# themayflyman/yet-another-raytracer

Hardware: NVIDIA B200
Metric: Mrays/s (primary+secondary) on david.obj 1920x1080 max-depth 50 (higher is better)
Workload: dtype f64

## Files before the change

### yet-another-raytracer_b200/csrc/device_trace.cuh

```cuda
#pragma once
#include "device_common.cuh"

namespace yart {

#ifndef YART_TRACE_THREADS
#define YART_TRACE_THREADS 128
#endif
constexpr int kTraceThreads = YART_TRACE_THREADS;
constexpr uint32_t kSentinel = 0x7FFFFFFFu;


YART_DEV bool sphere_t(D3 center, double radius, D3 ro, D3 rd, double t_min, double t_max, double& t) {
  D3 oc = ro - center;
  double a = length_squared(rd);
  double half_b = dot(oc, rd);
  double c = length_squared(oc) - radius * radius;
  double disc = half_b * half_b - a * c;
  if (disc < 0.0) return false;
  t = (0.0 - half_b - sqrt(disc)) / a;
  if (t < t_min || t_max < t) {
    t = (0.0 - half_b + sqrt(disc)) / a;
    if (t < t_min || t_max < t) return false;
  }
  return true;
// ... 219 lines not shown
  const float4* nodes;
  const float4* tris;
  const float4* leafgeo;
  const uint4* cnodes;
  float corigin[3], cscale;
  uint32_t root;
  uint32_t obj_index;
  uint32_t wrap;
  uint32_t refill_threshold;
  uint32_t node_threshold;
  uint32_t _pad;
  uint32_t n_nodes, n_tris;
  double sin_theta, cos_theta, offset[3];
  double bound[3];
  uint32_t* work_counter;
  unsigned long long* counters;
};

struct AnalyticParams {
  PassCommon c;
  DevScene scene;
  const yart_object* objects;
  uint32_t obj_begin, obj_end;
  const double* ray_time;
  uint64_t seed;
  uint32_t bounce;
  uint32_t spp_batch;
  uint32_t sample_base;
  uint32_t pixel_base;
  uint32_t media_mask;
  uint32_t _pad;
};

YART_DEV double min_nn(double a, double b) { return a < b ? a : b; }
YART_DEV double max_nn(double a, double b) { return a > b ? a : b; }

template <bool NEAR>
__device__ __noinline__ uint32_t box4_ieee(const float4* nd, double ox, double oy, double oz, double ix, double iy,
                                           double iz, double t_min, double t_best) {
  const float4 mnx = __ldg(nd + 0), mny = __ldg(nd + 2), mnz = __ldg(nd + 4);
  const float4 mxx = __ldg(nd + 1), mxy = __ldg(nd + 3), mxz = __ldg(nd + 5);
  uint32_t hitmask = 0;
#define YART_BOX(K, LX, LY, LZ, HX, HY, HZ)                                        \
  {                                                                                \
    double t0 = ((double)(LX) - ox) * ix, t1 = ((double)(HX) - ox) * ix;           \
    double tn = fmax(t_min, fmin(t0, t1));                                         \
    double tf = fmin(NEAR ? d_inf() : t_best, fmax(t0, t1));                       \
    t0 = ((double)(LY) - oy) * iy; t1 = ((double)(HY) - oy) * iy;                  \
    tn = fmax(tn, fmin(t0, t1)); tf = fmin(tf, fmax(t0, t1));                      \
    t0 = ((double)(LZ) - oz) * iz; t1 = ((double)(HZ) - oz) * iz;                  \
    tn = fmax(tn, fmin(t0, t1)); tf = fmin(tf, fmax(t0, t1));                      \
    const bool h = NEAR ? ((tf > tn) && (t_best >= tn)) : (tf > tn);               \
    hitmask |= h ? (1u << (K)) : 0u;                                               \
  }
  YART_BOX(0, mnx.x, mny.x, mnz.x, mxx.x, mxy.x, mxz.x)
  YART_BOX(1, mnx.y, mny.y, mnz.y, mxx.y, mxy.y, mxz.y)
  YART_BOX(2, mnx.z, mny.z, mnz.z, mxx.z, mxy.z, mxz.z)
  YART_BOX(3, mnx.w, mny.w, mnz.w, mxx.w, mxy.w, mxz.w)
#undef YART_BOX
  return hitmask;
}

#ifndef YART_TRAVERSE_MIN_BLOCKS
#define YART_TRAVERSE_MIN_BLOCKS 4
#endif

// ... 95 lines not shown
        }
        cur_used = 0;
        nxt_stage = 0;
        nxt_cnt = 0;
        if (!dyn_done) {
          if (lane == 0) claim_raw = atomicAdd(P.work_counter, 32u);
          nxt_stage = 1;
        }
        const uint32_t rank2 = rank - take1;
        const uint32_t take2 = min(need - take1, cur_cnt);
        const uint32_t id2 = __shfl_sync(0xffffffffu, id_cur, rank2 & 31u);
        if (fetching && !got && rank2 < take2) {
          new_id = id2;
          got = true;
        }
        cur_used = take2;
        if (fetching && !got) exhausted = true;
      } else if (nxt_stage == 1) {
        const uint64_t nb = dyn_base + __shfl_sync(0xffffffffu, claim_raw, 0);
        nxt_cnt = nb < n_items ? (uint32_t)min((unsigned long long)32, (unsigned long long)(n_items - nb)) : 0u;
        id_nxt = YART_MISS;
        if (lane < nxt_cnt) id_nxt = P.c.queue ? P.c.queue[nb + lane] : (uint32_t)(nb + lane);
        if (nxt_cnt < 32u) dyn_done = true;
        nxt_stage = 2;
      }
      if (got) {
        {
          ray_id = new_id;
          YART_CHECK(ray_id < P.c.n_rays);
          D3 ro, rd;
          if (P.c.rays32) load_ray_f32(P.c.rays32 + ray_id, ro, rd);
          else load_ray(P.c.rays + ray_id, ro, rd);
          t_best = P.c.first_pass ? P.c.t_max : fmin(P.c.hits[ray_id].t, P.c.t_max);
          if (NEAR) t_best = just_below(t_best);
          if (P.wrap & YART_WRAP_TRANSLATE) ro = ro - d3(P.offset[0], P.offset[1], P.offset[2]);
          if (P.wrap & YART_WRAP_ROTATE_Y) {
            const double ct = P.cos_theta, st = P.sin_theta;
            D3 org = ro, dir = rd;
            org.x = ct * ro.x - st * ro.z;
            org.z = st * ro.x + ct * ro.z;
            dir.x = ct * rd.x - st * rd.z;
            dir.z = st * rd.x + ct * rd.z;
            ro = org;
            rd = dir;
          }
          ox = ro.x; oy = ro.y; oz = ro.z;
          dx = rd.x; dy = rd.y; dz = rd.z;
          ix = 1.0 / dx; iy = 1.0 / dy; iz = 1.0 / dz;
          pos = (dx >= 0.0 ? 1u : 0u) | (dy >= 0.0 ? 2u : 0u) | (dz >= 0.0 ? 4u : 0u);
          sgn = NEAR ? (pos ^ 7u) : pos;
          if (!(isfinite(ix) && isfinite(iy) && isfinite(iz) && isfinite(ox) && isfinite(oy) && isfinite(oz))) pos |= 8u;
          if (MIXED) {
            ixf = (float)ix; iyf = (float)iy; izf = (float)iz;
            cxf = (float)(-(ox * ix)); cyf = (float)(-(oy * iy)); czf = (float)(-(oz * iz));
            const double a = fmax(fmax((P.bound[0] + fabs(ox)) * fabs(ix), (P.bound[1] + fabs(oy)) * fabs(iy)),
                                  (P.bound[2] + fabs(oz)) * fabs(iz));
            amax2 = __double2float_ru(a * (1.0 / 4194304.0));
            const float lo = 1e-30f, hi = 1e30f;
            const bool ok = fabsf(ixf) > lo && fabsf(ixf) < hi && fabsf(iyf) > lo && fabsf(iyf) < hi && fabsf(izf) > lo &&
                            fabsf(izf) < hi && fabsf(cxf) < hi && fabsf(cyf) < hi && fabsf(czf) < hi && amax2 < hi;
            if (!ok) pos |= 8u;
            t_best_f = (float)t_best;
          }
          cur = P.root;
          sp = 0;
          best_prim = YART_MISS;
          best_bu = best_bv = 0.0;
// ... 180 lines not shown
    YART_CHECK(ray_id < P.c.n_rays);
    D3 wo, wd;
    if (P.c.rays32) load_ray_f32(P.c.rays32 + ray_id, wo, wd);
    else load_ray(P.c.rays + ray_id, wo, wd);
    DevHit h;
    if (P.c.first_pass) {
      h.t = d_inf(); h.bu = 0.0; h.bv = 0.0; h.obj = YART_MISS; h.prim = 0;
    } else {
      h = P.c.hits[ray_id];
    }
    double t_best = fmin(h.t, P.c.t_max);
    bool changed = P.c.first_pass != 0;
    Rng rng;
    if (P.media_mask) rng = make_rng(P.seed, P.pixel_base + ray_id / P.spp_batch, P.sample_base + ray_id % P.spp_batch);
    else rng = make_rng(0, 0, 0);
    const double time = P.ray_time ? P.ray_time[ray_id] : 0.0;
    for (uint32_t oi = P.obj_begin; oi < P.obj_end; ++oi) {
      const yart_object& o = P.objects[oi];
      double t, bu = 0.0, bv = 0.0;
      uint32_t prim = 0;
      bool hit;
      if (o.kind == YART_OBJ_SPHERE && o.wrap == 0)
        hit = sphere_t(d3(o.p[0], o.p[1], o.p[2]), o.p[3], wo, wd, P.c.t_min, t_best, t);
      else
        hit = object_hit_t(P.scene, o, oi, wo, wd, time, P.c.t_min, t_best, rng, P.bounce, t, prim, bu, bv);
      if (hit) {
        t_best = t; h.t = t; h.obj = oi; h.prim = prim; h.bu = bu; h.bv = bv;
        changed = true;
      }
    }
    if (changed) P.c.hits[ray_id] = h;
  }
}
#endif

}
```

### yet-another-raytracer_b200/csrc/device_trace_lean.cu

```cuda
#define YART_TRACE_NO_ANALYTIC_KERNEL
#include "device_trace.cuh"

namespace yart {

template <bool NEAR, int STACK, int MIN_BLOCKS, bool COMPACT>
__global__ void __launch_bounds__(kTraceThreads, MIN_BLOCKS) k_traverse_lean(const TraverseParams P) {
  constexpr bool MIXED = true;
  __shared__ uint32_t s_stack[STACK + 1][kTraceThreads];
  __shared__ double s_ray[6][kTraceThreads];
  __shared__ double s_buv[2][kTraceThreads];
  const int tid = threadIdx.x;
  const uint32_t lane = tid & 31;
  const uint32_t n_items = P.c.n_items_dev ? *P.c.n_items_dev : (uint32_t)P.c.n_items;
  const uint32_t warp_global = (blockIdx.x * kTraceThreads + tid) >> 5;
  const uint32_t total_warps = gridDim.x * (kTraceThreads / 32);
  const uint32_t rpw = max(1u, min(32u, (uint32_t)(((uint64_t)n_items + total_warps - 1) / total_warps)));
  const uint32_t dyn_base = total_warps * rpw;
  if ((uint64_t)warp_global * rpw >= n_items) return;
  const uint32_t cur_base = warp_global * rpw;
  struct {
    uint32_t cur_cnt : 6, cur_used : 6, nxt_cnt : 6, nxt_stage : 2, dyn_done : 1;
  } w;
  w.cur_cnt = min(rpw, n_items - cur_base);
  w.cur_used = 0;
// ... 80 lines not shown
        }
        w.cur_used = 0;
        w.nxt_stage = 0;
        w.nxt_cnt = 0;
        if (!w.dyn_done) {
          if (lane == 0) claim_raw = atomicAdd(P.work_counter, 32u);
          w.nxt_stage = 1;
        }
        const uint32_t rank2 = rank - take1;
        const uint32_t take2 = min(need - take1, (uint32_t)w.cur_cnt);
        const uint32_t id2 = __shfl_sync(0xffffffffu, id_cur, rank2 & 31u);
        if (fetching && !got && rank2 < take2) {
          new_id = id2;
          got = true;
        }
        w.cur_used = take2;
        if (fetching && !got) exhausted = true;
      } else if (w.nxt_stage == 1) {
        const uint64_t nb = (uint64_t)dyn_base + __shfl_sync(0xffffffffu, claim_raw, 0);
        w.nxt_cnt = nb < n_items ? min(32u, n_items - (uint32_t)nb) : 0u;
        id_nxt = YART_MISS;
        if (lane < w.nxt_cnt) id_nxt = P.c.queue ? P.c.queue[nb + lane] : (uint32_t)(nb + lane);
        if (w.nxt_cnt < 32u) w.dyn_done = 1;
        w.nxt_stage = 2;
      }
      if (got) {
        {
          ray_id = new_id;
          YART_CHECK(ray_id < P.c.n_rays);
          D3 ro, rd;
          if (P.c.rays32) load_ray_f32(P.c.rays32 + ray_id, ro, rd);
          else load_ray(P.c.rays + ray_id, ro, rd);
          t_best = P.c.first_pass ? P.c.t_max : fmin(P.c.hits[ray_id].t, P.c.t_max);
          if (NEAR) t_best = just_below(t_best);
          if (P.wrap & YART_WRAP_TRANSLATE) ro = ro - d3(P.offset[0], P.offset[1], P.offset[2]);
          if (P.wrap & YART_WRAP_ROTATE_Y) {
            const double ct = P.cos_theta, st = P.sin_theta;
            D3 org = ro, dir = rd;
            org.x = ct * ro.x - st * ro.z;
            org.z = st * ro.x + ct * ro.z;
            dir.x = ct * rd.x - st * rd.z;
            dir.z = st * rd.x + ct * rd.z;
            ro = org;
            rd = dir;
          }
          const double ox = ro.x, oy = ro.y, oz = ro.z, dx = rd.x, dy = rd.y, dz = rd.z;
          const double ix = 1.0 / dx, iy = 1.0 / dy, iz = 1.0 / dz;
          s_ray[0][tid] = ox; s_ray[1][tid] = oy; s_ray[2][tid] = oz;
          s_ray[3][tid] = dx; s_ray[4][tid] = dy; s_ray[5][tid] = dz;
          pos = (dx >= 0.0 ? 1u : 0u) | (dy >= 0.0 ? 2u : 0u) | (dz >= 0.0 ? 4u : 0u);
          sgn = NEAR ? (pos ^ 7u) : pos;
          if (!(isfinite(ix) && isfinite(iy) && isfinite(iz) && isfinite(ox) && isfinite(oy) && isfinite(oz))) pos |= 8u;
          if (MIXED) {
            ixf = (float)ix; iyf = (float)iy; izf = (float)iz;
            cxf = (float)(-(ox * ix)); cyf = (float)(-(oy * iy)); czf = (float)(-(oz * iz));
            const double a = fmax(fmax((P.bound[0] + fabs(ox)) * fabs(ix), (P.bound[1] + fabs(oy)) * fabs(iy)),
                                  (P.bound[2] + fabs(oz)) * fabs(iz));
            amax2 = __double2float_ru(a * (1.0 / 4194304.0));
            const float lo = 1e-30f, hi = 1e30f;
            const bool ok = fabsf(ixf) > lo && fabsf(ixf) < hi && fabsf(iyf) > lo && fabsf(iyf) < hi && fabsf(izf) > lo &&
                            fabsf(izf) < hi && fabsf(cxf) < hi && fabsf(cyf) < hi && fabsf(czf) < hi && amax2 < hi;
            if (!ok) pos |= 8u;
            if (COMPACT) {
              const float ax = P.cscale * ixf, ay = P.cscale * iyf, az = P.cscale * izf;
              const float bx = fmaf(-8388608.f, ax, fmaf(P.corigin[0], ixf, cxf));
              const float by = fmaf(-8388608.f, ay, fmaf(P.corigin[1], iyf, cyf));
              const float bz = fmaf(-8388608.f, az, fmaf(P.corigin[2], izf, czf));
// ... 242 lines not shown
```

### yet-another-raytracer_b200/csrc/yart_device.cu

```cuda
#include <algorithm>
#include <cfloat>
#include <cmath>
#include <cstdio>
#include <cstdlib>
#include <cstring>
#include <map>
#include <numeric>
#include <string>
#include <vector>

#include "../../include/yart_spectral_tables.h"
#include "device_build.h"
#include "device_shade.cuh"
#include "host_common.h"

namespace yart {

__global__ void __launch_bounds__(256) k_export(const DevScene S, const yart_ray* rays, const DevHit* hits, yart_hit* out_hits,
                                                 uint64_t n) {
  for (uint64_t i = blockIdx.x * (uint64_t)blockDim.x + threadIdx.x; i < n; i += (uint64_t)gridDim.x * blockDim.x) {
    const DevHit h = hits[i];
    yart_hit out;
    if (h.obj == YART_MISS) {
      out.t = d_inf(); out.u = 0.0; out.v = 0.0; out.prim_id = YART_MISS; out.obj_id = YART_MISS; out.front_face = 0;
// ... 299 lines not shown
    nd.pad[0] = nd.pad[1] = nd.pad[2] = 0;
    nodes.push_back(nd);
    id = (uint32_t)nodes.size() - 1;
    return merge(merge(bx[0], bx[1]), merge(bx[2], bx[3]));
  }
};

}
}

using namespace yart;

struct yart_ctx {
  int device = 0;
  int sm_count = 148;
  cudaStream_t stream = nullptr;
  bool own_stream = true;
  std::string err;

  bool have_scene = false;
  std::vector<void*> scene_allocs;
  DevScene scene;
  yart_object* d_solo = nullptr;
  std::map<const void*, int> traverse_blocks;
  std::vector<yart_object> h_objects;
  std::vector<DevMesh> h_meshes;
  uint32_t n_meshes = 0;
  uint32_t max_stack = 0;
  bool has_media = false;
  uint32_t builder = YART_BUILDER_DEVICE;
  double* d_cie = nullptr;
  double* d_smits = nullptr;

  DevBuf rays, hits_export, time, wavelength, throughput, hits, queue_a, queue_b, counts, work, counters, film, rgba;
  cudaEvent_t ev0 = nullptr, ev1 = nullptr;
  std::vector<cudaEvent_t> ev_pool;
  cudaStream_t copy_in = nullptr, copy_out = nullptr;
  std::vector<cudaEvent_t> chunk_events;

  void free_scene() {
    for (void* p : scene_allocs) cudaFree(p);
    scene_allocs.clear();
    have_scene = false;
    d_solo = nullptr;
  }
};

namespace yart {
cudaStream_t ctx_stream(yart_ctx* ctx) { return ctx->stream; }
int ctx_device(const yart_ctx* ctx) { return ctx->device; }
void ctx_set_error(yart_ctx* ctx, const std::string& msg) { ctx->err = msg; }
}

namespace {

template <class T>
int upload(yart_ctx* ctx, const T* host, size_t n, T** out) {
  *out = nullptr;
  if (n == 0) return YART_OK;
  void* p = nullptr;
  CUDA_TRY(ctx, cudaMalloc(&p, n * sizeof(T)));
  ctx->scene_allocs.push_back(p);
  CUDA_TRY(ctx, cudaMemcpyAsync(p, host, n * sizeof(T), cudaMemcpyHostToDevice, ctx->stream));
  *out = reinterpret_cast<T*>(p);
  return YART_OK;
}

DevCamera make_camera(const yart_camera& c) {
  auto sub = [](const double* a, const double* b, double* o) { for (int i = 0; i < 3; ++i) o[i] = a[i] - b[i]; };
  auto unit = [](double* a) {
    double l = std::sqrt(a[0] * a[0] + a[1] * a[1] + a[2] * a[2]);
// ... 34 lines not shown

typedef void (*TraverseKernel)(const TraverseParams);
}
namespace yart {
TraverseKernel lean_traverse_kernel(bool near, uint32_t max_stack, int ctas_per_sm, bool compact);
}
namespace {
template <bool MIXED>
TraverseKernel pick_traverse_kernel_m(bool near, bool count, uint32_t max_stack) {
  if (max_stack <= 32) {
    if (near) return count ? k_traverse<true, true, 32, MIXED> : k_traverse<true, false, 32, MIXED>;
    return count ? k_traverse<false, true, 32, MIXED> : k_traverse<false, false, 32, MIXED>;
  }
  if (near) return count ? k_traverse<true, true, 64, MIXED> : k_traverse<true, false, 64, MIXED>;
  return count ? k_traverse<false, true, 64, MIXED> : k_traverse<false, false, 64, MIXED>;
}
TraverseKernel pick_traverse_kernel(bool near, bool count, uint32_t max_stack, bool mixed) {
  return mixed ? pick_traverse_kernel_m<true>(near, count, max_stack) : pick_traverse_kernel_m<false>(near, count, max_stack);
}

struct QueryArgs {
  PassCommon c;
  const yart_object* d_objects;
  const yart_object* h_objects;
  uint32_t n_objects;
  const double* ray_time;
  uint64_t seed;
  uint32_t bounce, spp_batch, sample_base, pixel_base;
  uint32_t* work_counters;
  unsigned long long* counters;
  bool near, count;
};

int run_passes(yart_ctx* ctx, const QueryArgs& q, uint64_t* launches) {
  static const int rt = tune_env("YART_TUNE_RT", 8), nt = tune_env("YART_TUNE_NT", 12);
  static const int carve = tune_env("YART_TUNE_CARVEOUT", 35);
  static const int carve_lean = tune_env("YART_TUNE_CARVEOUT_LEAN", 50);
  static const int mixed = tune_env("YART_TUNE_MIXED", 1);
  bool first = true;
  uint32_t i = 0, n_trav = 0;
  auto is_mesh = [&](uint32_t k) {
    return q.h_objects[k].kind == YART_OBJ_MESH && !(q.h_objects[k].wrap & YART_WRAP_MEDIUM);
  };
  if (q.n_objects == 0) {
    AnalyticParams A;
    memset(&A, 0, sizeof(A));
    A.c = q.c;
    A.c.first_pass = 1;
    A.scene = ctx->scene;
    A.objects = q.d_objects;
    A.spp_batch = 1;
    k_analytic<<<ctx->sm_count * 8, 256, 0, ctx->stream>>>(A);
    if (launches) (*launches)++;
  }
  while (i < q.n_objects) {
    if (is_mesh(i)) {
      const yart_object& o = q.h_objects[i];
      const DevMesh& m = ctx->h_meshes[o.index];
      TraverseParams T;
      memset(&T, 0, sizeof(T));
      T.c = q.c;
      T.c.first_pass = first ? 1u : 0u;
      T.nodes = m.nodes;
      T.tris = m.tris;
      T.leafgeo = m.leafgeo;
      T.cnodes = m.cnodes;
      T.cscale = m.cscale;
      for (int k = 0; k < 3; ++k) T.corigin[k] = m.corigin[k];
      T.root = m.root;
      T.n_nodes = m.n_nodes;
      T.n_tris = m.n_tris;
      T.obj_index = i;
      T.wrap = o.wrap & (YART_WRAP_ROTATE_Y | YART_WRAP_TRANSLATE);
      T.refill_threshold = (uint32_t)std::max(1, std::min(32, rt));
      T.node_threshold = (uint32_t)std::max(1, std::min(32, nt));
      T.sin_theta = o.sin_theta;
      T.cos_theta = o.cos_theta;
      for (int k = 0; k < 3; ++k) T.offset[k] = o.offset[k];
      T.work_counter = q.work_counters + n_trav++;
      T.counters = q.counters;
      for (int k = 0; k < 3; ++k) T.bound[k] = m.bound[k];
      static const int lean = tune_env("YART_TUNE_LEAN", 5);
      static const int lean_stack24 = tune_env("YART_TUNE_LEAN_STACK24", 1);
      static const int lean_ref = tune_env("YART_TUNE_LEAN_REF", 0);
      const bool use_lean = lean && mixed && !q.count && (q.near || lean_ref);
      TraverseKernel k = use_lean ? yart::lean_traverse_kernel(q.near, (lean_stack24 || ctx->max_stack > 24) ? ctx->max_stack : 25u, lean,
                                                                 m.cnodes != nullptr && q.near)
                                  : pick_traverse_kernel(q.near, q.count, ctx->max_stack, mixed != 0);
      int& per_sm = ctx->traverse_blocks[(const void*)k];
      if (per_sm == 0) {
        cudaFuncSetAttribute(reinterpret_cast<const void*>(k), cudaFuncAttributePreferredSharedMemoryCarveout, use_lean ? carve_lean : carve);
        CUDA_TRY(ctx, cudaOccupancyMaxActiveBlocksPerMultiprocessor(&per_sm, reinterpret_cast<const void*>(k), kTraceThreads, 0));
        per_sm = std::max(per_sm, 1);
      }
      k<<<per_sm * ctx->sm_count, kTraceThreads, 0, ctx->stream>>>(T);
      i++;
    } else {
      uint32_t j = i;
      while (j < q.n_objects && !is_mesh(j)) ++j;
      AnalyticParams A;
      memset(&A, 0, sizeof(A));
      A.c = q.c;
      A.c.first_pass = first ? 1u : 0u;
      A.scene = ctx->scene;
      A.objects = q.d_objects;
      A.obj_begin = i;
      A.obj_end = j;
      A.ray_time = q.ray_time;
      A.seed = q.seed;
      A.bounce = q.bounce;
      A.spp_batch = q.spp_batch ? q.spp_batch : 1;
      A.sample_base = q.sample_base;
      A.pixel_base = q.pixel_base;
      A.media_mask = ctx->has_media ? 1u : 0u;
      k_analytic<<<ctx->sm_count * 8, 256, 0, ctx->stream>>>(A);
      i = j;
    }
    first = false;
    if (launches) (*launches)++;
  }
  CUDA_TRY(ctx, cudaGetLastError());
  return YART_OK;
}

}

extern "C" {

int yart_device_count(void) {
  int n = 0;
  if (cudaGetDeviceCount(&n) != cudaSuccess) return 0;
  return n;
}

int yart_ctx_create(int device, yart_ctx** out) {
  if (!out) {
    set_global_error("yart_ctx_create: null argument");
    return YART_ERR_INVALID;
  }
  int n = 0;
  cudaError_t e = cudaGetDeviceCount(&n);
  if (e != cudaSuccess || n <= 0) {
    set_global_error(std::string("no CUDA device: ") + (e != cudaSuccess ? cudaGetErrorString(e) : "device count is 0") +
                     " (this library has no CPU fallback)");
    return YART_ERR_CUDA;
  }
  if (device < 0 || device >= n) {
    set_global_error("yart_ctx_create: device index out of range");
    return YART_ERR_INVALID;
  }
  cudaDeviceProp prop;
  if ((e = cudaSetDevice(device)) != cudaSuccess || (e = cudaGetDeviceProperties(&prop, device)) != cudaSuccess) {
// ... 4 lines not shown
    set_global_error("this library is built for sm_100a (B200) only; device is sm_" + std::to_string(prop.major) +
                     std::to_string(prop.minor));
    return YART_ERR_CUDA;
  }
  yart_ctx* ctx = new yart_ctx();
  ctx->device = device;
  ctx->sm_count = prop.multiProcessorCount;
  if ((e = cudaStreamCreateWithFlags(&ctx->stream, cudaStreamNonBlocking)) != cudaSuccess ||
      (e = cudaEventCreate(&ctx->ev0)) != cudaSuccess || (e = cudaEventCreate(&ctx->ev1)) != cudaSuccess ||
      (e = cudaMalloc((void**)&ctx->d_cie, sizeof(double) * 3 * YART_N_CIE)) != cudaSuccess ||
      (e = cudaMalloc((void**)&ctx->d_smits, sizeof(double) * 7 * YART_N_BINS)) != cudaSuccess) {
    set_global_error(std::string("context setup: ") + cudaGetErrorString(e));
    delete ctx;
    return YART_ERR_CUDA;
  }
  if ((e = cudaMemcpy(ctx->d_cie, YART_CIE_X, sizeof(double) * YART_N_CIE, cudaMemcpyHostToDevice)) != cudaSuccess ||
      (e = cudaMemcpy(ctx->d_cie + YART_N_CIE, YART_CIE_Y, sizeof(double) * YART_N_CIE, cudaMemcpyHostToDevice)) != cudaSuccess ||
      (e = cudaMemcpy(ctx->d_cie + 2 * YART_N_CIE, YART_CIE_Z, sizeof(double) * YART_N_CIE, cudaMemcpyHostToDevice)) != cudaSuccess ||
      (e = cudaMemcpy(ctx->d_smits, YART_SMITS_BASIS, sizeof(double) * 7 * YART_N_BINS, cudaMemcpyHostToDevice)) != cudaSuccess) {
    set_global_error(std::string("context setup (spectral tables): ") + cudaGetErrorString(e));
    yart_ctx_destroy(ctx);
    return YART_ERR_CUDA;
  }
  *out = ctx;
  return YART_OK;
}

void yart_ctx_destroy(yart_ctx* ctx) {
  if (!ctx) return;
  cudaSetDevice(ctx->device);
  cudaDeviceSynchronize();
  ctx->free_scene();
  DevBuf* bufs[] = {&ctx->rays, &ctx->hits_export, &ctx->time, &ctx->wavelength, &ctx->throughput, &ctx->hits,
                    &ctx->queue_a, &ctx->queue_b, &ctx->counts, &ctx->work, &ctx->counters, &ctx->film, &ctx->rgba};
  for (DevBuf* b : bufs) b->release();
  for (cudaEvent_t e : ctx->ev_pool) cudaEventDestroy(e);
  for (cudaEvent_t e : ctx->chunk_events) cudaEventDestroy(e);
  if (ctx->copy_in) cudaStreamDestroy(ctx->copy_in);
  if (ctx->copy_out) cudaStreamDestroy(ctx->copy_out);
  if (ctx->ev0) cudaEventDestroy(ctx->ev0);
  if (ctx->ev1) cudaEventDestroy(ctx->ev1);
  if (ctx->d_cie) cudaFree(ctx->d_cie);
  if (ctx->d_smits) cudaFree(ctx->d_smits);
  if (ctx->own_stream && ctx->stream) cudaStreamDestroy(ctx->stream);
  delete ctx;
}

const char* yart_last_error(const yart_ctx* ctx) { return ctx ? ctx->err.c_str() : yart_last_error_global(); }

int yart_ctx_set_stream(yart_ctx* ctx, void* cuda_stream) {
  if (!ctx) return YART_ERR_INVALID;
  CUDA_TRY(ctx, cudaSetDevice(ctx->device));
  if (ctx->stream || !ctx->own_stream) CUDA_TRY(ctx, cudaStreamSynchronize(ctx->stream));
  if (ctx->own_stream && ctx->stream) cudaStreamDestroy(ctx->stream);
  ctx->stream = reinterpret_cast<cudaStream_t>(cuda_stream);
  ctx->own_stream = false;
  return YART_OK;
}

int yart_host_register(yart_ctx* ctx, void* ptr, uint64_t bytes) {
  if (!ctx) return YART_ERR_INVALID;
  if (!ptr || !bytes) {
    ctx->err = "yart_host_register: null pointer or zero size";
    return YART_ERR_INVALID;
  }
  CUDA_TRY(ctx, cudaSetDevice(ctx->device));
  const cudaError_t e = cudaHostRegister(ptr, (size_t)bytes, cudaHostRegisterPortable);
  if (e != cudaSuccess) {
    cudaGetLastError();
    ctx->err = std::string("yart_host_register: ") + cudaGetErrorString(e);
// ... 378 lines not shown
  const char* fn = f32 ? "yart_closest_hit_f32" : "yart_closest_hit";
  if (!ctx->have_scene) {
    ctx->err = std::string(fn) + ": no scene (call yart_ctx_set_scene first)";
    return YART_ERR_INVALID;
  }
  if ((n && (!rays || !hits)) || n > 0xFFFFFFF0ull || order > YART_ORDER_NEAR) {
    ctx->err = std::string(fn) + ": bad argument";
    return YART_ERR_INVALID;
  }
  const uintptr_t ray_align = f32 ? 7u : 15u, hit_align = f32 ? 3u : 7u;
  if ((flags & YART_FLAG_DEVICE_PTRS) && ((reinterpret_cast<uintptr_t>(rays) & ray_align) || (reinterpret_cast<uintptr_t>(hits) & hit_align))) {
    ctx->err = std::string(fn) + (f32 ? ": device ray arrays must be 8-byte aligned (hits: 4)" : ": device ray arrays must be 16-byte aligned (hits: 8)");
    return YART_ERR_INVALID;
  }
  if (target != YART_TARGET_WORLD && target >= ctx->n_meshes) {
    ctx->err = std::string(fn) + ": target is neither a mesh index nor YART_TARGET_WORLD";
    return YART_ERR_INVALID;
  }
  CUDA_TRY(ctx, cudaSetDevice(ctx->device));
  if (stats) memset(stats, 0, sizeof(*stats));
  if (n == 0) return YART_OK;
  const size_t ray_bytes = f32 ? sizeof(yart_ray_f32) : sizeof(yart_ray), hit_bytes = f32 ? sizeof(yart_hit_f32) : sizeof(yart_hit);
  const bool dev = (flags & YART_FLAG_DEVICE_PTRS) != 0;
  const bool count = (flags & YART_FLAG_COUNT_VISITS) != 0;
  const char* d_rays = static_cast<const char*>(rays);
  char* d_hits = static_cast<char*>(hits);
  if (!dev) {
    CUDA_TRY(ctx, ctx->rays.reserve(n * ray_bytes));
    CUDA_TRY(ctx, ctx->hits_export.reserve(n * hit_bytes));
    d_rays = ctx->rays.as<char>();
    d_hits = ctx->hits_export.as<char>();
  }
  const uint32_t n_list = (target == YART_TARGET_WORLD) ? ctx->scene.n_objects : 1u;
  const size_t work_bytes = ((size_t)n_list + 2) * sizeof(uint32_t);
  CUDA_TRY(ctx, ctx->work.reserve(work_bytes));
  CUDA_TRY(ctx, ctx->counters.reserve(64));
  CUDA_TRY(ctx, ctx->hits.reserve(n * sizeof(DevHit)));
  CUDA_TRY(ctx, cudaMemsetAsync(ctx->counters.p, 0, 64, ctx->stream));

  yart_object solo;
  memset(&solo, 0, sizeof(solo));
  solo.kind = YART_OBJ_MESH;
  solo.cos_theta = 1.0;
  QueryArgs q;
  memset(&q, 0, sizeof(q));
  q.c.t_min = t_min;
  q.c.t_max = t_max;
  DevScene export_scene = ctx->scene;
  if (target == YART_TARGET_WORLD) {
    q.d_objects = ctx->scene.objects;
    q.h_objects = ctx->h_objects.data();
    q.n_objects = ctx->scene.n_objects;
  } else {
    solo.index = target;
    q.d_objects = ctx->d_solo + target;
    q.h_objects = &solo;
    q.n_objects = 1;
    export_scene.objects = ctx->d_solo + target;
  }
  q.seed = 0;
  q.bounce = 1;
  q.spp_batch = 1;
  q.work_counters = ctx->work.as<uint32_t>();
  q.counters = ctx->counters.as<unsigned long long>();
  q.near = order == YART_ORDER_NEAR;
  q.count = count;
  uint64_t launches = 0;
// ... 183 lines not shown
  }
  return YART_OK;
  YART_ABI_GUARD_END(ctx, "yart_dump_path_rays")
}

static int render_impl(yart_ctx* ctx, const yart_camera* cam, const yart_render_opts* o, double* film_xyz, yart_stats* stats,
                       yart_ray* dump_out, uint64_t dump_cap) {
  if (!ctx->have_scene || !cam || !o) {
    ctx->err = "yart_render: missing scene or null argument";
    return YART_ERR_INVALID;
  }
  CUDA_TRY(ctx, cudaSetDevice(ctx->device));
  RenderParams R;
  int rc = fill_render_params(ctx, cam, o, R);
  if (rc) return rc;
  if (stats) memset(stats, 0, sizeof(*stats));
  const uint32_t n_pixels_total = o->width * o->height;
  const uint32_t n_samples = o->sample_end - o->sample_begin;
  const bool dumping = film_xyz == nullptr;
  const bool dev = !dumping && (o->flags & YART_FLAG_DEVICE_PTRS) != 0;
  const size_t film_bytes = (size_t)n_pixels_total * 3 * sizeof(double);
  double* d_film = film_xyz;
  CUDA_TRY(ctx, cudaEventRecord(ctx->ev0, ctx->stream));
  if (!dev) {
    CUDA_TRY(ctx, ctx->film.reserve(film_bytes));
    d_film = ctx->film.as<double>();
    if (dumping) CUDA_TRY(ctx, cudaMemsetAsync(d_film, 0, film_bytes, ctx->stream));
    else CUDA_TRY(ctx, cudaMemcpyAsync(d_film, film_xyz, film_bytes, cudaMemcpyHostToDevice, ctx->stream));
  }
  uint64_t total_rays = 0, total_paths = 0, launches = 0, trace_launches = 0;
  double trace_ms = 0.0;
  uint32_t deepest = 0;
  if (n_samples > 0) {
    static const int max_paths_log2 = std::max(10, std::min(30, tune_env("YART_TUNE_MAX_PATHS_LOG2", 28)));
    uint64_t kMaxPaths = 1ull << max_paths_log2;
    {
      const uint64_t kStateBytesPerPath = sizeof(yart_ray) + 3 * sizeof(double) + sizeof(DevHit) + 2 * sizeof(uint32_t);
      size_t free_b = 0, total_b = 0;
      CUDA_TRY(ctx, cudaMemGetInfo(&free_b, &total_b));
      const DevBuf* held[] = {&ctx->rays, &ctx->time, &ctx->wavelength, &ctx->throughput, &ctx->hits, &ctx->queue_a, &ctx->queue_b};
      uint64_t avail = free_b;
      for (const DevBuf* b : held) avail += b->cap;
      const uint64_t margin = (256ull << 20) + (dev ? 0 : film_bytes);
      const uint64_t fit = avail > margin ? (avail - margin) / kStateBytesPerPath : 0;
      kMaxPaths = std::min<uint64_t>(kMaxPaths, fit);
      static const int mem_cap_mb = tune_env("YART_TUNE_STATE_MB", 0);
      if (mem_cap_mb > 0) kMaxPaths = std::min<uint64_t>(kMaxPaths, ((uint64_t)mem_cap_mb << 20) / kStateBytesPerPath);
      if (kMaxPaths < 1024) {
        ctx->err = "yart_render: not enough free device memory for the path state (" + std::to_string(free_b >> 20) +
                   " MiB free of " + std::to_string(total_b >> 20) + " MiB; 112 bytes per path in flight)";
        return YART_ERR_NOMEM;
      }
    }
    uint32_t spp_batch = o->batch_spp ? o->batch_spp : (uint32_t)std::max<uint64_t>(1, kMaxPaths / n_pixels_total);
    spp_batch = std::min(spp_batch, n_samples);
    uint32_t pix_chunk = n_pixels_total;
    if ((uint64_t)pix_chunk * spp_batch > kMaxPaths) pix_chunk = (uint32_t)std::max<uint64_t>(1, kMaxPaths / spp_batch);
    const uint64_t cap = (uint64_t)pix_chunk * spp_batch;
    CUDA_TRY(ctx, ctx->rays.reserve(cap * sizeof(yart_ray)));
    CUDA_TRY(ctx, ctx->time.reserve(cap * sizeof(double)));
    CUDA_TRY(ctx, ctx->wavelength.reserve(cap * sizeof(double)));
    CUDA_TRY(ctx, ctx->throughput.reserve(cap * sizeof(double)));
    CUDA_TRY(ctx, ctx->hits.reserve(cap * sizeof(DevHit)));
    CUDA_TRY(ctx, ctx->queue_a.reserve(cap * sizeof(uint32_t)));
    CUDA_TRY(ctx, ctx->queue_b.reserve(cap * sizeof(uint32_t)));
    const uint32_t D = o->max_depth;
    const size_t n_counts = (size_t)D + 2;
    const size_t n_obj_slots = (size_t)ctx->scene.n_objects + 1;
    const size_t n_work = n_obj_slots * D;
    CUDA_TRY(ctx, ctx->counts.reserve(n_counts * sizeof(uint32_t)));
    CUDA_TRY(ctx, ctx->work.reserve(n_work * sizeof(uint32_t)));
    while (ctx->ev_pool.size() < 2 * (size_t)D) {
      cudaEvent_t e;
      CUDA_TRY(ctx, cudaEventCreate(&e));
      ctx->ev_pool.push_back(e);
    }
    R.st.rays = ctx->rays.as<yart_ray>();
    R.st.time = ctx->time.as<double>();
    R.st.wavelength = ctx->wavelength.as<double>();
    R.st.throughput = ctx->throughput.as<double>();
    R.st.hits = ctx->hits.as<DevHit>();
    uint32_t* counts = ctx->counts.as<uint32_t>();
    uint32_t* work = ctx->work.as<uint32_t>();
    std::vector<uint32_t> h_counts(n_counts);
    const bool near = o->order == YART_ORDER_NEAR;
    const bool count = (o->flags & YART_FLAG_COUNT_VISITS) != 0;
    const int stream_grid = ctx->sm_count * 8;
    CUDA_TRY(ctx, ctx->counters.reserve(64));
    CUDA_TRY(ctx, cudaMemsetAsync(ctx->counters.p, 0, 64, ctx->stream));

    for (uint32_t s0 = o->sample_begin; s0 < o->sample_end; s0 += spp_batch) {
      const uint32_t spp = std::min(spp_batch, o->sample_end - s0);
      for (uint32_t p0 = 0; p0 < n_pixels_total; p0 += pix_chunk) {
        R.pixel_base = p0;
        R.n_pixels = std::min(pix_chunk, n_pixels_total - p0);
        R.sample_base = s0;
        R.spp_batch = spp;
        CUDA_TRY(ctx, cudaMemsetAsync(counts, 0, n_counts * sizeof(uint32_t), ctx->stream));
        CUDA_TRY(ctx, cudaMemsetAsync(work, 0, n_work * sizeof(uint32_t), ctx->stream));
        uint32_t* qa = ctx->queue_a.as<uint32_t>();
        uint32_t* qb = ctx->queue_b.as<uint32_t>();
// ... 206 lines not shown
```

Baseline: 1355.

## Bin rays by nearest mesh instance and trace each bin on its own stream

Adds a k_order kernel that tests each ray against the root boxes of every mesh instance and scatters the ray into a per-instance sub-queue for the instance whose box it enters first. Each sub-queue then runs the full set of object passes, starting with its likely-nearest instance. The aim is an early, tight t_best that prunes traversal of the other instances, and the sub-queues run concurrently on side streams. A tie_wins check keeps hit ownership deterministic when a later-index object re-tests a ray, at the cost of an extra hits load per ray. The path only engages for near-order queries with two to eight mesh instances and no media, and it needs extra per-path queue memory.

New measurement: 1286, median of 6. 5.1% lower.

```diff
diff --git a/yet-another-raytracer_b200/csrc/device_trace.cuh b/yet-another-raytracer_b200/csrc/device_trace.cuh
--- a/yet-another-raytracer_b200/csrc/device_trace.cuh
+++ b/yet-another-raytracer_b200/csrc/device_trace.cuh
@@ -275,6 +275,28 @@
   uint32_t _pad;
 };
 
+constexpr uint32_t kMaxOrdered = 8;
+struct OrderInstance {
+  const float4* nodes;
+  uint32_t root;
+  uint32_t wrap;
+  double sin_theta, cos_theta, offset[3];
+};
+struct OrderParams {
+  PassCommon c;
+  OrderInstance inst[kMaxOrdered];
+  uint32_t n_inst;
+  uint32_t stride;
+  uint32_t* sub;
+  uint32_t* sub_count;
+};
+
+YART_DEV bool tie_wins(const TraverseParams& P, uint32_t ray_id) {
+  if (P.c.first_pass) return false;
+  const uint32_t holder = P.c.hits[ray_id].obj;
+  return holder > P.obj_index && holder != YART_MISS;
+}
+
 YART_DEV double min_nn(double a, double b) { return a < b ? a : b; }
 YART_DEV double max_nn(double a, double b) { return a > b ? a : b; }
 
@@ -436,7 +458,7 @@
           if (P.c.rays32) load_ray_f32(P.c.rays32 + ray_id, ro, rd);
           else load_ray(P.c.rays + ray_id, ro, rd);
           t_best = P.c.first_pass ? P.c.t_max : fmin(P.c.hits[ray_id].t, P.c.t_max);
-          if (NEAR) t_best = just_below(t_best);
+          if (NEAR && !tie_wins(P, ray_id)) t_best = just_below(t_best);
           if (P.wrap & YART_WRAP_TRANSLATE) ro = ro - d3(P.offset[0], P.offset[1], P.offset[2]);
           if (P.wrap & YART_WRAP_ROTATE_Y) {
             const double ct = P.cos_theta, st = P.sin_theta;
@@ -683,6 +705,81 @@
     if (changed) P.c.hits[ray_id] = h;
   }
 }
+
+constexpr int kOrderThreads = 256;
+__global__ void __launch_bounds__(kOrderThreads) k_order(const OrderParams P) {
+  __shared__ uint32_t s_cnt[kOrderThreads / 32][kMaxOrdered];
+  __shared__ uint32_t s_base[kMaxOrdered];
+  const uint64_t n = P.c.n_items_dev ? (uint64_t)*P.c.n_items_dev : P.c.n_items;
+  const uint32_t lane = threadIdx.x & 31, warp = threadIdx.x >> 5;
+  for (uint64_t tile = (uint64_t)blockIdx.x * kOrderThreads; tile < n; tile += (uint64_t)gridDim.x * kOrderThreads) {
+    const uint64_t item = tile + threadIdx.x;
+    const bool active = item < n;
+    uint32_t ray_id = 0, g = 0;
+    if (active) {
+      ray_id = P.c.queue ? P.c.queue[item] : (uint32_t)item;
+      YART_CHECK(ray_id < P.c.n_rays);
+      D3 wo, wd;
+      if (P.c.rays32) load_ray_f32(P.c.rays32 + ray_id, wo, wd);
+      else load_ray(P.c.rays + ray_id, wo, wd);
+      double first = d_inf();
+      for (uint32_t k = 0; k < P.n_inst; ++k) {
+        const OrderInstance& in = P.inst[k];
+        D3 ro = wo, rd = wd;
+        if (in.wrap & YART_WRAP_TRANSLATE) ro = ro - d3(in.offset[0], in.offset[1], in.offset[2]);
+        if (in.wrap & YART_WRAP_ROTATE_Y) {
+          const double ct = in.cos_theta, st = in.sin_theta;
+          const D3 org = ro, dir = rd;
+          ro.x = ct * org.x - st * org.z;
+          ro.z = st * org.x + ct * org.z;
+          rd.x = ct * dir.x - st * dir.z;
+          rd.z = st * dir.x + ct * dir.z;
+        }
+        double t = P.c.t_min;
+        if (in.root < 0x80000000u) {
+          const float4* nd = in.nodes + (size_t)in.root * 8;
+          const float4 mnx = __ldg(nd + 0), mxx = __ldg(nd + 1), mny = __ldg(nd + 2), mxy = __ldg(nd + 3),
+                       mnz = __ldg(nd + 4), mxz = __ldg(nd + 5);
+          const float lo[4][3] = {{mnx.x, mny.x, mnz.x}, {mnx.y, mny.y, mnz.y}, {mnx.z, mny.z, mnz.z}, {mnx.w, mny.w, mnz.w}};
+          const float hi[4][3] = {{mxx.x, mxy.x, mxz.x}, {mxx.y, mxy.y, mxz.y}, {mxx.z, mxy.z, mxz.z}, {mxx.w, mxy.w, mxz.w}};
+          const double ix = 1.0 / rd.x, iy = 1.0 / rd.y, iz = 1.0 / rd.z;
+          t = d_inf();
+#pragma unroll
+          for (int c = 0; c < 4; ++c) {
+            double t0 = ((double)lo[c][0] - ro.x) * ix, t1 = ((double)hi[c][0] - ro.x) * ix;
+            double tn = fmax(P.c.t_min, fmin(t0, t1)), tf = fmax(t0, t1);
+            t0 = ((double)lo[c][1] - ro.y) * iy; t1 = ((double)hi[c][1] - ro.y) * iy;
+            tn = fmax(tn, fmin(t0, t1)); tf = fmin(tf, fmax(t0, t1));
+            t0 = ((double)lo[c][2] - ro.z) * iz; t1 = ((double)hi[c][2] - ro.z) * iz;
+            tn = fmax(tn, fmin(t0, t1)); tf = fmin(tf, fmax(t0, t1));
+            if (tf >= tn && tn < t) t = tn;
+          }
+        }
+        if (t < first) { first = t; g = k; }
+      }
+    }
+    uint32_t mine = 0;
+    for (uint32_t k = 0; k < P.n_inst; ++k) {
+      const uint32_t m = __ballot_sync(0xffffffffu, active && g == k);
+      if (g == k) mine = m;
+      if (lane == 0) s_cnt[warp][k] = (uint32_t)__popc(m);
+    }
+    __syncthreads();
+    if (threadIdx.x < P.n_inst) {
+      uint32_t total = 0;
+      for (int w = 0; w < kOrderThreads / 32; ++w) total += s_cnt[w][threadIdx.x];
+      s_base[threadIdx.x] = total ? atomicAdd(P.sub_count + threadIdx.x, total) : 0u;
+    }
+    __syncthreads();
+    if (active) {
+      uint32_t slot = s_base[g] + __popc(mine & ((1u << lane) - 1u));
+      for (uint32_t w = 0; w < warp; ++w) slot += s_cnt[w][g];
+      YART_CHECK(slot < P.stride);
+      P.sub[(size_t)g * P.stride + slot] = ray_id;
+    }
+    __syncthreads();
+  }
+}
 #endif
 
 }
diff --git a/yet-another-raytracer_b200/csrc/device_trace_lean.cu b/yet-another-raytracer_b200/csrc/device_trace_lean.cu
--- a/yet-another-raytracer_b200/csrc/device_trace_lean.cu
+++ b/yet-another-raytracer_b200/csrc/device_trace_lean.cu
@@ -136,7 +136,7 @@
           if (P.c.rays32) load_ray_f32(P.c.rays32 + ray_id, ro, rd);
           else load_ray(P.c.rays + ray_id, ro, rd);
           t_best = P.c.first_pass ? P.c.t_max : fmin(P.c.hits[ray_id].t, P.c.t_max);
-          if (NEAR) t_best = just_below(t_best);
+          if (NEAR && !tie_wins(P, ray_id)) t_best = just_below(t_best);
           if (P.wrap & YART_WRAP_TRANSLATE) ro = ro - d3(P.offset[0], P.offset[1], P.offset[2]);
           if (P.wrap & YART_WRAP_ROTATE_Y) {
             const double ct = P.cos_theta, st = P.sin_theta;
diff --git a/yet-another-raytracer_b200/csrc/yart_device.cu b/yet-another-raytracer_b200/csrc/yart_device.cu
--- a/yet-another-raytracer_b200/csrc/yart_device.cu
+++ b/yet-another-raytracer_b200/csrc/yart_device.cu
@@ -355,11 +355,13 @@
   double* d_cie = nullptr;
   double* d_smits = nullptr;
 
-  DevBuf rays, hits_export, time, wavelength, throughput, hits, queue_a, queue_b, counts, work, counters, film, rgba;
+  DevBuf rays, hits_export, time, wavelength, throughput, hits, queue_a, queue_b, order_queue, counts, work, counters, film, rgba;
   cudaEvent_t ev0 = nullptr, ev1 = nullptr;
   std::vector<cudaEvent_t> ev_pool;
   cudaStream_t copy_in = nullptr, copy_out = nullptr;
   std::vector<cudaEvent_t> chunk_events;
+  std::vector<cudaStream_t> side_streams;
+  std::vector<cudaEvent_t> side_events;
 
   void free_scene() {
     for (void* p : scene_allocs) cudaFree(p);
@@ -460,92 +462,168 @@
   bool near, count;
 };
 
+bool is_mesh_pass(const yart_object& o) { return o.kind == YART_OBJ_MESH && !(o.wrap & YART_WRAP_MEDIUM); }
+
+std::vector<uint32_t> ordered_instances(const yart_ctx* ctx, const yart_object* objects, uint32_t n_objects, bool near) {
+  std::vector<uint32_t> inst;
+  if (!near || ctx->has_media) return inst;
+  for (uint32_t i = 0; i < n_objects; ++i)
+    if (is_mesh_pass(objects[i])) inst.push_back(i);
+  if (inst.size() < 2 || inst.size() > kMaxOrdered) inst.clear();
+  return inst;
+}
+
+size_t pass_slots(uint32_t n_objects, size_t n_ordered) {
+  return std::max<size_t>(n_objects, n_ordered * n_ordered + n_ordered) + 2;
+}
+
 int run_passes(yart_ctx* ctx, const QueryArgs& q, uint64_t* launches) {
   static const int rt = tune_env("YART_TUNE_RT", 8), nt = tune_env("YART_TUNE_NT", 12);
   static const int carve = tune_env("YART_TUNE_CARVEOUT", 35);
   static const int carve_lean = tune_env("YART_TUNE_CARVEOUT_LEAN", 50);
   static const int mixed = tune_env("YART_TUNE_MIXED", 1);
-  bool first = true;
-  uint32_t i = 0, n_trav = 0;
-  auto is_mesh = [&](uint32_t k) {
-    return q.h_objects[k].kind == YART_OBJ_MESH && !(q.h_objects[k].wrap & YART_WRAP_MEDIUM);
+  uint32_t n_trav = 0;
+  auto is_mesh = [&](uint32_t k) { return is_mesh_pass(q.h_objects[k]); };
+  auto mesh_pass = [&](const PassCommon& c, uint32_t i, bool first, cudaStream_t stream) {
+    const yart_object& o = q.h_objects[i];
+    const DevMesh& m = ctx->h_meshes[o.index];
+    TraverseParams T;
+    memset(&T, 0, sizeof(T));
+    T.c = c;
+    T.c.first_pass = first ? 1u : 0u;
+    T.nodes = m.nodes;
+    T.tris = m.tris;
+    T.leafgeo = m.leafgeo;
+    T.cnodes = m.cnodes;
+    T.cscale = m.cscale;
+    for (int k = 0; k < 3; ++k) T.corigin[k] = m.corigin[k];
+    T.root = m.root;
+    T.n_nodes = m.n_nodes;
+    T.n_tris = m.n_tris;
+    T.obj_index = i;
+    T.wrap = o.wrap & (YART_WRAP_ROTATE_Y | YART_WRAP_TRANSLATE);
+    T.refill_threshold = (uint32_t)std::max(1, std::min(32, rt));
+    T.node_threshold = (uint32_t)std::max(1, std::min(32, nt));
+    T.sin_theta = o.sin_theta;
+    T.cos_theta = o.cos_theta;
+    for (int k = 0; k < 3; ++k) T.offset[k] = o.offset[k];
+    T.work_counter = q.work_counters + n_trav++;
+    T.counters = q.counters;
+    for (int k = 0; k < 3; ++k) T.bound[k] = m.bound[k];
+    static const int lean = tune_env("YART_TUNE_LEAN", 5);
+    static const int lean_stack24 = tune_env("YART_TUNE_LEAN_STACK24", 1);
+    static const int lean_ref = tune_env("YART_TUNE_LEAN_REF", 0);
+    const bool use_lean = lean && mixed && !q.count && (q.near || lean_ref);
+    TraverseKernel k = use_lean ? yart::lean_traverse_kernel(q.near, (lean_stack24 || ctx->max_stack > 24) ? ctx->max_stack : 25u, lean,
+                                                               m.cnodes != nullptr && q.near)
+                                : pick_traverse_kernel(q.near, q.count, ctx->max_stack, mixed != 0);
+    int& per_sm = ctx->traverse_blocks[(const void*)k];
+    if (per_sm == 0) {
+      cudaFuncSetAttribute(reinterpret_cast<const void*>(k), cudaFuncAttributePreferredSharedMemoryCarveout, use_lean ? carve_lean : carve);
+      CUDA_TRY(ctx, cudaOccupancyMaxActiveBlocksPerMultiprocessor(&per_sm, reinterpret_cast<const void*>(k), kTraceThreads, 0));
+      per_sm = std::max(per_sm, 1);
+    }
+    k<<<per_sm * ctx->sm_count, kTraceThreads, 0, stream>>>(T);
+    if (launches) (*launches)++;
+    return YART_OK;
   };
-  if (q.n_objects == 0) {
+  auto analytic_pass = [&](const PassCommon& c, uint32_t i, uint32_t j, bool first, cudaStream_t stream) {
     AnalyticParams A;
     memset(&A, 0, sizeof(A));
-    A.c = q.c;
-    A.c.first_pass = 1;
+    A.c = c;
+    A.c.first_pass = first ? 1u : 0u;
     A.scene = ctx->scene;
     A.objects = q.d_objects;
-    A.spp_batch = 1;
-    k_analytic<<<ctx->sm_count * 8, 256, 0, ctx->stream>>>(A);
+    A.obj_begin = i;
+    A.obj_end = j;
+    A.ray_time = q.ray_time;
+    A.seed = q.seed;
+    A.bounce = q.bounce;
+    A.spp_batch = q.spp_batch ? q.spp_batch : 1;
+    A.sample_base = q.sample_base;
+    A.pixel_base = q.pixel_base;
+    A.media_mask = ctx->has_media ? 1u : 0u;
+    k_analytic<<<ctx->sm_count * 8, 256, 0, stream>>>(A);
     if (launches) (*launches)++;
-  }
-  while (i < q.n_objects) {
-    if (is_mesh(i)) {
-      const yart_object& o = q.h_objects[i];
+  };
+  constexpr uint32_t kNone = 0xFFFFFFFFu;
+  auto passes = [&](const PassCommon& c, uint32_t lead, cudaStream_t stream) {
+    bool first = true;
+    if (lead != kNone) {
+      const int rc = mesh_pass(c, lead, true, stream);
+      if (rc) return rc;
+      first = false;
+    }
+    uint32_t i = 0;
+    while (i < q.n_objects) {
+      if (i == lead) {
+        i++;
+      } else if (is_mesh(i)) {
+        const int rc = mesh_pass(c, i, first, stream);
+        if (rc) return rc;
+        i++;
+        first = false;
+      } else {
+        uint32_t j = i;
+        while (j < q.n_objects && !is_mesh(j)) ++j;
+        analytic_pass(c, i, j, first, stream);
+        i = j;
+        first = false;
+      }
+    }
+    return (int)YART_OK;
+  };
+  if (q.n_objects == 0) analytic_pass(q.c, 0, 0, true, ctx->stream);
+  const std::vector<uint32_t> inst = ordered_instances(ctx, q.h_objects, q.n_objects, q.near);
+  if (inst.empty()) {
+    const int rc = passes(q.c, kNone, ctx->stream);
+    if (rc) return rc;
+  } else {
+    const uint32_t M = (uint32_t)inst.size();
+    CUDA_TRY(ctx, ctx->order_queue.reserve((size_t)M * q.c.n_rays * sizeof(uint32_t)));
+    OrderParams O;
+    memset(&O, 0, sizeof(O));
+    O.c = q.c;
+    O.n_inst = M;
+    O.stride = q.c.n_rays;
+    O.sub = ctx->order_queue.as<uint32_t>();
+    O.sub_count = q.work_counters + M * M;
+    for (uint32_t g = 0; g < M; ++g) {
+      const yart_object& o = q.h_objects[inst[g]];
       const DevMesh& m = ctx->h_meshes[o.index];
-      TraverseParams T;
-      memset(&T, 0, sizeof(T));
-      T.c = q.c;
-      T.c.first_pass = first ? 1u : 0u;
-      T.nodes = m.nodes;
-      T.tris = m.tris;
-      T.leafgeo = m.leafgeo;
-      T.cnodes = m.cnodes;
-      T.cscale = m.cscale;
-      for (int k = 0; k < 3; ++k) T.corigin[k] = m.corigin[k];
-      T.root = m.root;
-      T.n_nodes = m.n_nodes;
-      T.n_tris = m.n_tris;
-      T.obj_index = i;
-      T.wrap = o.wrap & (YART_WRAP_ROTATE_Y | YART_WRAP_TRANSLATE);
-      T.refill_threshold = (uint32_t)std::max(1, std::min(32, rt));
-      T.node_threshold = (uint32_t)std::max(1, std::min(32, nt));
-      T.sin_theta = o.sin_theta;
-      T.cos_theta = o.cos_theta;
-      for (int k = 0; k < 3; ++k) T.offset[k] = o.offset[k];
-      T.work_counter = q.work_counters + n_trav++;
-      T.counters = q.counters;
-      for (int k = 0; k < 3; ++k) T.bound[k] = m.bound[k];
-      static const int lean = tune_env("YART_TUNE_LEAN", 5);
-      static const int lean_stack24 = tune_env("YART_TUNE_LEAN_STACK24", 1);
-      static const int lean_ref = tune_env("YART_TUNE_LEAN_REF", 0);
-      const bool use_lean = lean && mixed && !q.count && (q.near || lean_ref);
-      TraverseKernel k = use_lean ? yart::lean_traverse_kernel(q.near, (lean_stack24 || ctx->max_stack > 24) ? ctx->max_stack : 25u, lean,
-                                                                 m.cnodes != nullptr && q.near)
-                                  : pick_traverse_kernel(q.near, q.count, ctx->max_stack, mixed != 0);
-      int& per_sm = ctx->traverse_blocks[(const void*)k];
-      if (per_sm == 0) {
-        cudaFuncSetAttribute(reinterpret_cast<const void*>(k), cudaFuncAttributePreferredSharedMemoryCarveout, use_lean ? carve_lean : carve);
-        CUDA_TRY(ctx, cudaOccupancyMaxActiveBlocksPerMultiprocessor(&per_sm, reinterpret_cast<const void*>(k), kTraceThreads, 0));
-        per_sm = std::max(per_sm, 1);
-      }
-      k<<<per_sm * ctx->sm_count, kTraceThreads, 0, ctx->stream>>>(T);
-      i++;
-    } else {
-      uint32_t j = i;
-      while (j < q.n_objects && !is_mesh(j)) ++j;
-      AnalyticParams A;
-      memset(&A, 0, sizeof(A));
-      A.c = q.c;
-      A.c.first_pass = first ? 1u : 0u;
-      A.scene = ctx->scene;
-      A.objects = q.d_objects;
-      A.obj_begin = i;
-      A.obj_end = j;
-      A.ray_time = q.ray_time;
-      A.seed = q.seed;
-      A.bounce = q.bounce;
-      A.spp_batch = q.spp_batch ? q.spp_batch : 1;
-      A.sample_base = q.sample_base;
-      A.pixel_base = q.pixel_base;
-      A.media_mask = ctx->has_media ? 1u : 0u;
-      k_analytic<<<ctx->sm_count * 8, 256, 0, ctx->stream>>>(A);
-      i = j;
-    }
-    first = false;
+      O.inst[g].nodes = m.nodes;
+      O.inst[g].root = m.root;
+      O.inst[g].wrap = o.wrap & (YART_WRAP_ROTATE_Y | YART_WRAP_TRANSLATE);
+      O.inst[g].sin_theta = o.sin_theta;
+      O.inst[g].cos_theta = o.cos_theta;
+      for (int k = 0; k < 3; ++k) O.inst[g].offset[k] = o.offset[k];
+    }
+    k_order<<<ctx->sm_count * 8, kOrderThreads, 0, ctx->stream>>>(O);
     if (launches) (*launches)++;
+    while (ctx->side_streams.size() + 1 < M) {
+      cudaStream_t st;
+      CUDA_TRY(ctx, cudaStreamCreateWithFlags(&st, cudaStreamNonBlocking));
+      ctx->side_streams.push_back(st);
+    }
+    while (ctx->side_events.size() < M) {
+      cudaEvent_t e;
+      CUDA_TRY(ctx, cudaEventCreateWithFlags(&e, cudaEventDisableTiming));
+      ctx->side_events.push_back(e);
+    }
+    CUDA_TRY(ctx, cudaEventRecord(ctx->side_events[0], ctx->stream));
+    for (uint32_t g = 0; g < M; ++g) {
+      const cudaStream_t st = g == 0 ? ctx->stream : ctx->side_streams[g - 1];
+      if (g > 0) CUDA_TRY(ctx, cudaStreamWaitEvent(st, ctx->side_events[0], 0));
+      PassCommon c = q.c;
+      c.queue = O.sub + (size_t)g * O.stride;
+      c.n_items_dev = O.sub_count + g;
+      const int rc = passes(c, inst[g], st);
+      if (rc) return rc;
+    }
+    for (uint32_t g = 1; g < M; ++g) {
+      CUDA_TRY(ctx, cudaEventRecord(ctx->side_events[g], ctx->side_streams[g - 1]));
+      CUDA_TRY(ctx, cudaStreamWaitEvent(ctx->stream, ctx->side_events[g], 0));
+    }
   }
   CUDA_TRY(ctx, cudaGetLastError());
   return YART_OK;
@@ -616,10 +694,12 @@
   cudaDeviceSynchronize();
   ctx->free_scene();
   DevBuf* bufs[] = {&ctx->rays, &ctx->hits_export, &ctx->time, &ctx->wavelength, &ctx->throughput, &ctx->hits,
-                    &ctx->queue_a, &ctx->queue_b, &ctx->counts, &ctx->work, &ctx->counters, &ctx->film, &ctx->rgba};
+                    &ctx->queue_a, &ctx->queue_b, &ctx->order_queue, &ctx->counts, &ctx->work, &ctx->counters, &ctx->film, &ctx->rgba};
   for (DevBuf* b : bufs) b->release();
   for (cudaEvent_t e : ctx->ev_pool) cudaEventDestroy(e);
   for (cudaEvent_t e : ctx->chunk_events) cudaEventDestroy(e);
+  for (cudaEvent_t e : ctx->side_events) cudaEventDestroy(e);
+  for (cudaStream_t st : ctx->side_streams) cudaStreamDestroy(st);
   if (ctx->copy_in) cudaStreamDestroy(ctx->copy_in);
   if (ctx->copy_out) cudaStreamDestroy(ctx->copy_out);
   if (ctx->ev0) cudaEventDestroy(ctx->ev0);
@@ -1064,7 +1144,8 @@
     d_hits = ctx->hits_export.as<char>();
   }
   const uint32_t n_list = (target == YART_TARGET_WORLD) ? ctx->scene.n_objects : 1u;
-  const size_t work_bytes = ((size_t)n_list + 2) * sizeof(uint32_t);
+  const size_t n_ordered = target == YART_TARGET_WORLD ? ordered_instances(ctx, ctx->h_objects.data(), n_list, order == YART_ORDER_NEAR).size() : 0;
+  const size_t work_bytes = pass_slots(n_list, n_ordered) * sizeof(uint32_t);
   CUDA_TRY(ctx, ctx->work.reserve(work_bytes));
   CUDA_TRY(ctx, ctx->counters.reserve(64));
   CUDA_TRY(ctx, ctx->hits.reserve(n * sizeof(DevHit)));
@@ -1314,13 +1395,14 @@
   double trace_ms = 0.0;
   uint32_t deepest = 0;
   if (n_samples > 0) {
+    const size_t n_ordered = ordered_instances(ctx, ctx->h_objects.data(), R.tail_begin, o->order == YART_ORDER_NEAR).size();
     static const int max_paths_log2 = std::max(10, std::min(30, tune_env("YART_TUNE_MAX_PATHS_LOG2", 28)));
     uint64_t kMaxPaths = 1ull << max_paths_log2;
     {
-      const uint64_t kStateBytesPerPath = sizeof(yart_ray) + 3 * sizeof(double) + sizeof(DevHit) + 2 * sizeof(uint32_t);
+      const uint64_t kStateBytesPerPath = sizeof(yart_ray) + 3 * sizeof(double) + sizeof(DevHit) + (2 + n_ordered) * sizeof(uint32_t);
       size_t free_b = 0, total_b = 0;
       CUDA_TRY(ctx, cudaMemGetInfo(&free_b, &total_b));
-      const DevBuf* held[] = {&ctx->rays, &ctx->time, &ctx->wavelength, &ctx->throughput, &ctx->hits, &ctx->queue_a, &ctx->queue_b};
+      const DevBuf* held[] = {&ctx->rays, &ctx->time, &ctx->wavelength, &ctx->throughput, &ctx->hits, &ctx->queue_a, &ctx->queue_b, &ctx->order_queue};
       uint64_t avail = free_b;
       for (const DevBuf* b : held) avail += b->cap;
       const uint64_t margin = (256ull << 20) + (dev ? 0 : film_bytes);
@@ -1330,7 +1412,7 @@
       if (mem_cap_mb > 0) kMaxPaths = std::min<uint64_t>(kMaxPaths, ((uint64_t)mem_cap_mb << 20) / kStateBytesPerPath);
       if (kMaxPaths < 1024) {
         ctx->err = "yart_render: not enough free device memory for the path state (" + std::to_string(free_b >> 20) +
-                   " MiB free of " + std::to_string(total_b >> 20) + " MiB; 112 bytes per path in flight)";
+                   " MiB free of " + std::to_string(total_b >> 20) + " MiB; " + std::to_string(kStateBytesPerPath) + " bytes per path in flight)";
         return YART_ERR_NOMEM;
       }
     }
@@ -1346,9 +1428,10 @@
     CUDA_TRY(ctx, ctx->hits.reserve(cap * sizeof(DevHit)));
     CUDA_TRY(ctx, ctx->queue_a.reserve(cap * sizeof(uint32_t)));
     CUDA_TRY(ctx, ctx->queue_b.reserve(cap * sizeof(uint32_t)));
+    CUDA_TRY(ctx, ctx->order_queue.reserve(cap * n_ordered * sizeof(uint32_t)));
     const uint32_t D = o->max_depth;
     const size_t n_counts = (size_t)D + 2;
-    const size_t n_obj_slots = (size_t)ctx->scene.n_objects + 1;
+    const size_t n_obj_slots = pass_slots(R.tail_begin, n_ordered);
     const size_t n_work = n_obj_slots * D;
     CUDA_TRY(ctx, ctx->counts.reserve(n_counts * sizeof(uint32_t)));
     CUDA_TRY(ctx, ctx->work.reserve(n_work * sizeof(uint32_t)));
```
